# Vi-Sri/CerebralSignalNetworks

Hardware: AMD Instinct MI355X
Metric: EEG-segments/sec training (128ch x 500, hidden=768) (higher is better)
Workload: dtype bf16

## Files before the change

### cerebralsignalnetworks_amd/cabi.py

```python
import ctypes
import os

import torch

_HERE = os.path.dirname(os.path.abspath(__file__))
LIB_PATH = os.environ.get("CSN_LIB_PATH") or os.path.join(_HERE, "lib", "libcsn_hip.so")

CSN_F32, CSN_BF16 = 0, 1
STATUS_TIMEOUT, STATUS_NONFINITE, STATUS_STALE_SLOT = 1, 2, 4
ABI_VERSION = 6
LSTM_STATE = 0x100
LSTM_DROPOUT = 0x200
LSTM_REVERSE = 0x400
LSTM_RESIDENT = 0x800
RESIDENT_MAX_H = 128
TOPK_MERGE_STAGED_MAX = 2048
GRAD_OVERWRITE, GRAD_ACCUMULATE = 0, 1
SEG_DECAYED, SEG_SCALED = 1, 2

_c_void_p, _c_int, _c_i64, _c_size_t, _c_float = (ctypes.c_void_p, ctypes.c_int, ctypes.c_int64,
                                                  ctypes.c_size_t, ctypes.c_float)
_c_double = ctypes.c_double


# ... 410 lines not shown
        _check(load().csn_lstm_plan_set_io(self._plan, int(y_all_pitch), int(dy_all_pitch), int(bool(dx_add))))
        self._io = (int(y_all_pitch), int(dy_all_pitch), bool(dx_add))

    def _pitched(self, t, pitch, name):
        d = self.desc
        _need_cuda(t)
        pitch = pitch or d.H
        if (t.dtype != torch.float32 or tuple(t.shape) != (d.B, d.T, d.H) or t.stride() != (d.T * pitch, pitch, 1)
                or t.data_ptr() % 16):
            raise CsnError(f"LSTM {name}: a float32 [B,T,H] view with pitch {pitch} is needed, got {t.dtype} "
                           f"{tuple(t.shape)} strides {t.stride()}")
        return t

    def set_dropout(self, p, seed=0, subsequence=0):
        _check(load().csn_lstm_plan_set_dropout(self._plan, float(p), int(seed) & 0xFFFFFFFFFFFFFFFF,
                                                int(subsequence) & 0xFFFFFFFF))

    def dgates_copies(self):
        return load().csn_lstm_plan_dgates_copies(self._plan)

    def half_tile_launches(self, which):
        return load().csn_lstm_plan_half_tile_launches(self._plan, which)

    def forward(self, x_bti, w_ih, w_hh, b_ih, b_hh, want_all=False, h0=None, c0=None, want_state=False, y_all=None,
                state_out=None):
        d = self.desc
        _need_cuda(x_bti)
        if x_bti.dtype != torch.float32 or x_bti.stride(2) != 1:
            x_bti = x_bti.float().contiguous()
        want = (d.B, d.T, d.I) if self._views is None else self._views + (d.I,)
        assert x_bti.shape == want, (tuple(x_bti.shape), want)
        y_last = torch.empty((d.B, d.H), dtype=torch.float32, device=x_bti.device)
        if y_all is not None:
            y_all = self._pitched(y_all, self._io[0], "y_all")
        elif want_all:
            if self._io[0]:
                raise CsnError("LSTM y_all: the plan has a y_all pitch set (set_io): pass the view to write into")
            y_all = torch.empty((d.B, d.T, d.H), dtype=torch.float32, device=x_bti.device)
        ws = [[p.detach() for p in group] for group in (w_ih, w_hh, b_ih, b_hh)]
        for group in ws:
            for p in group:
                assert p.dtype == torch.float32 and p.is_contiguous() and p.is_cuda
        h0, c0 = self._state_in(h0), self._state_in(c0)
        if want_state and state_out is not None:
            h_n, c_n = state_out
            for out in state_out:
# ... 434 lines not shown
```

### cerebralsignalnetworks_amd/csrc/csn_common.h

```cpp
#pragma once
#include <hip/hip_runtime.h>
#include <stdint.h>
#include <stdio.h>
#include <stdlib.h>
#include <atomic>
#include <string>

#include "../../include/csn_hip.h"

namespace csn {

typedef __bf16 bf16_t;
typedef __attribute__((ext_vector_type(8))) __bf16 bf16x8;
typedef __attribute__((ext_vector_type(4))) __bf16 bf16x4;
typedef __attribute__((ext_vector_type(4))) float f32x4;
typedef __attribute__((ext_vector_type(4))) short s16x4;

void set_error(const std::string& msg);
int fail(int status, const char* fmt, ...);

#define CSN_HIP_CHECK(expr)                                                              \
  do {                                                                                   \
    hipError_t _e = (expr);                                                              \
    if (_e != hipSuccess)                                                                \
      return ::csn::fail(CSN_ERR_HIP, "%s failed: %s (%s:%d)", #expr, hipGetErrorString(_e), \
                         __FILE__, __LINE__);                                            \
  } while (0)

#define CSN_LAUNCH_CHECK()                                                               \
  do {                                                                                   \
    hipError_t _e = hipGetLastError();                                                   \
    if (_e != hipSuccess)                                                                \
      return ::csn::fail(CSN_ERR_HIP, "kernel launch failed: %s (%s:%d)",                \
                         hipGetErrorString(_e), __FILE__, __LINE__);                     \
  } while (0)

#define CSN_REQUIRE(cond, ...)                                                           \
  do {                                                                                   \
    if (!(cond)) return ::csn::fail(CSN_ERR_INVALID_ARGUMENT, __VA_ARGS__);              \
  } while (0)

struct Options {
  bool cell_v1, no_persist, no_persist_bwd, persist_streams, no_xcd_local, no_rotate, no_fuse_x, no_beside, beside_128,
      no_side_stream, fwd_ksplit, fwd_nsplit, fwd_flags, bwd_flags, dpoll_no_hint, fwd_hint, gemm_no_dma, gemm_no_256, gemm_generic, tn_no_tr, tn_no_stagger, filter_v1, tags_no_rearm, gemm_no_192, no_half_tiles, nt_no_w4, no_fwd_park;
  int chunk;
  int tn_stages;
};
static inline Options options_from_env() {
  auto on = [](const char* name) { return getenv(name) != nullptr; };
  auto num = [](const char* name, int dflt) {
    const char* e = getenv(name);
    return e ? atoi(e) : dflt;
  };
  Options o{};
  o.cell_v1 = on("CSN_CELL_V1");
  o.no_persist = on("CSN_NO_PERSIST");
  o.no_persist_bwd = on("CSN_NO_PERSIST_BWD");
  o.persist_streams = on("CSN_PERSIST_STREAMS");
  o.no_xcd_local = on("CSN_NO_XCD_LOCAL");
  o.no_rotate = on("CSN_NO_ROTATE");
  o.no_fuse_x = on("CSN_NO_FUSE_X");
  o.no_beside = on("CSN_NO_BESIDE");
  o.beside_128 = on("CSN_BESIDE_128");
  o.no_half_tiles = on("CSN_NO_HALF_TILES");
  o.no_fwd_park = on("CSN_NO_FWD_PARK");
  o.no_side_stream = on("CSN_NO_SIDE_STREAM");
  o.fwd_ksplit = on("CSN_FWD_KSPLIT");
  o.fwd_nsplit = on("CSN_FWD_NSPLIT");
  o.fwd_flags = on("CSN_FWD_FLAGS");
  o.bwd_flags = on("CSN_BWD_FLAGS");
  o.dpoll_no_hint = on("CSN_DPOLL_NO_HINT");
  o.fwd_hint = on("CSN_FWD_HINT");
  o.tn_no_stagger = on("CSN_TN_NO_STAGGER");
  o.gemm_no_dma = on("CSN_GEMM_NO_DMA");
  o.gemm_no_256 = on("CSN_GEMM_NO_256");
  o.gemm_no_192 = on("CSN_GEMM_NO_192");
  o.nt_no_w4 = on("CSN_NT_NO_W4");
  o.gemm_generic = on("CSN_GEMM_GENERIC");
  o.tn_no_tr = on("CSN_TN_NO_TR");
  o.filter_v1 = on("CSN_FILTER_V1");
#ifdef CSN_SLAB_TAGS
  o.tags_no_rearm = on("CSN_TAGS_NO_REARM");
#endif
  o.chunk = num("CSN_LSTM_CHUNK", 32);
  if (o.chunk < 1) o.chunk = 1;
  o.tn_stages = num("CSN_TN_STAGES", 4);
  return o;
}

static inline hipStream_t as_stream(csnStream_t s) { return reinterpret_cast<hipStream_t>(s); }
template <auto Kernel>
static int ensure_dyn_lds(int bytes) {
  static std::atomic<unsigned> done{0u};
// ... 68 lines not shown
```

### cerebralsignalnetworks_amd/csrc/lstm.hip

```cpp
#include <algorithm>
#include <cstring>
#include <vector>

#include "csn_common.h"
#include "lstm_cell_blk.h"
#include "lstm_cell_common.h"
#include "lstm_dropout.h"
#include "lstm_f32_persist.h"
#include "lstm_resident.h"

namespace csn {

struct LayerWs {
  size_t wih, whh, whht, wiht, whh_blk, whht_blk, bias, xproj, gates, c_all, h_all, dgates, dx, dc_carry, hblk[2],
      dgblk[2], h_blk_all, counters, dg_blk_all, bflags;
  size_t h_drop;
};
struct WsLayout {
  LayerWs layer[8];
  size_t x_c, x_blk, wih0_blk, dy_tm, tn_scratch, colsum, status, agree, agree_b, zeros_bh, f32_bias_part, total;
  size_t zero_fwd, zero_fwd_bytes, zero_bwd, zero_bwd_bytes;
  bool fuse_x;
  bool il, persist, persist_bwd;
  bool fwd_ns;
  bool f32_persist;
};

static bool whole_chip() {
  int dev = 0, cus = 0;
  if (hipGetDevice(&dev) != hipSuccess) return false;
  return hipDeviceGetAttribute(&cus, hipDeviceAttributeMultiprocessorCount, dev) == hipSuccess && cus >= 256;
}

static WsLayout make_layout(const csnLstmDesc& d, int training, bool dropout, const Options& opt) {
  WsLayout w{};
  w.il = cell_blk_supported(d.H, d.dtype, opt);
  const bool slabs_fit = ((size_t)d.T + 1) * (((size_t)d.B + 63) / 64 * 64) * (size_t)d.H * 8 < ((size_t)1 << 32);
  w.fwd_ns = w.il && fwd_ns_supported(d.B, d.H, d.dtype, opt) && d.L <= 4;
  w.persist = w.fwd_ns || (w.il && slabs_fit && fwd_persist_supported(d.B, d.H, d.dtype, opt) && d.L <= 4);
  w.persist_bwd = w.persist && slabs_fit && training && bwd_persist_supported(d.B, d.H, d.dtype, opt);
  size_t off = 0;
  const size_t es = dtype_size(d.dtype);
  auto take = [&](size_t bytes) {
// ... 56 lines not shown
    for (int l = 0; l < d.L; ++l) w.layer[l].h_blk_all = take(((size_t)d.T + 1) * Bpad * H * 4);
    if (training) {
      for (int l = 0; l < d.L; ++l) w.layer[l].dg_blk_all = take((size_t)d.T * Bpad * G * 4);
      w.zeros_bh = take((size_t)d.B * H * 4);
      w.f32_bias_part = take(MTt * 4 * G * 4);
      w.zero_bwd = off;
      for (int l = 0; l < d.L; ++l) w.layer[l].bflags = take((size_t)d.T * MTt * kF32FlagLine * 4);
      w.zero_bwd_bytes = off - w.zero_bwd;
    }
  }
  if (w.persist) {
    w.zero_fwd = off;
    for (int l = 0; l < d.L; ++l) w.layer[l].counters = take(((size_t)d.T + 1) * (Bpad / 64) * 4 * kPersistFlagLine * 4);
    w.agree = take(((size_t)d.T + 8) * 8 * sizeof(unsigned long long));
    w.zero_fwd_bytes = off - w.zero_fwd;
  }
  if (w.persist_bwd) {
    w.zero_bwd = off;
    for (int l = 0; l < d.L; ++l) {
      w.layer[l].dc_carry = take((size_t)d.B * H * 4);
      w.layer[l].bflags = take((size_t)d.T * (Bpad / 64) * 3 * kPersistFlagLine * 4);
    }
    w.agree_b = take(((size_t)d.T + 8) * 8 * sizeof(unsigned long long));
    w.zero_bwd_bytes = off - w.zero_bwd;
  }
  if (training) {
    w.dy_tm = take(TB * H * 4);
    w.tn_scratch = take(tn_bytes);
    w.colsum = take(colsum_scratch_bytes(G));
  }
  for (int l = 0; dropout && l + 1 < d.L; ++l) w.layer[l].h_drop = take(TB * H * es);
  w.total = off;
  return w;
}

static const int kPlanBits = CSN_LSTM_STATE | CSN_LSTM_DROPOUT | CSN_LSTM_REVERSE | CSN_LSTM_RESIDENT;

static int check_resident(const char* fn, const csnLstmDesc* d, int training) {
  if ((training & CSN_LSTM_RESIDENT) && !resident_supported(d->H))
    return fail(CSN_ERR_UNSUPPORTED, "%s: CSN_LSTM_RESIDENT takes H <= %d, not H=%d", fn, kResidentMaxH, d->H);
  return CSN_OK;
}
static void resident_options(Options& opt) {
  opt.cell_v1 = true;
  opt.no_persist = true;
}
// ... 259 lines not shown
  }
  CSN_HIP_CHECK(hipEventRecord(g_prof.pair[k][i], st));
  if (end) ++g_prof.pairs_used[k];
  return CSN_OK;
}

}

struct csnLstmPlan {
  csnLstmDesc d;
  int training;
  int dropout = 0;
  float drop_p = 0.f;
  uint64_t drop_seed = 0;
  uint32_t drop_subsequence = 0;
  int state;
  bool state_seen = false;
  int device;
  csn::Options opt;
  csn::WsLayout w;
  csn::SideCtx sc;
  csn::Prof prof;
  int dgates_copies = 0;
  int half_launches[2] = {0, 0};
  csnGradReadyFn grad_cb = nullptr;
  void* grad_cb_user = nullptr;
  int grad_accumulate = 0;
  int reverse = 0;
  int resident = 0;
  int64_t y_pitch = 0, dy_pitch = 0;
  int dx_add = 0;
  std::vector<int32_t> lengths;
  int t_eff = 0;
  int32_t* len_dev = nullptr;
  int32_t* len_pin = nullptr;
  hipEvent_t len_ev = nullptr;
  std::vector<int32_t> view_row, view_t0;
  int view_src_rows = 0, view_src_T = 0;
  int32_t* view_dev = nullptr;
  int32_t* view_pin = nullptr;
  hipEvent_t view_ev = nullptr;
  void grads_ready(int layer) const {
    if (grad_cb != nullptr) grad_cb(grad_cb_user, layer);
  }
};

// ... 41 lines not shown
    if (P->prof.ev[i]) (void)hipEventDestroy(P->prof.ev[i]);
  for (int k = 0; k < 2; ++k)
    for (hipEvent_t e : P->prof.pair[k]) (void)hipEventDestroy(e);
  if (P->len_ev) (void)hipEventDestroy(P->len_ev);
  if (P->len_pin) (void)hipHostFree(P->len_pin);
  if (P->len_dev) (void)hipFree(P->len_dev);
  if (P->view_ev) (void)hipEventDestroy(P->view_ev);
  if (P->view_pin) (void)hipHostFree(P->view_pin);
  if (P->view_dev) (void)hipFree(P->view_dev);
  if (switched) (void)hipSetDevice(cur);
  delete P;
}

extern "C" size_t csn_lstm_plan_workspace_bytes(const csnLstmPlan* P) { return P ? P->w.total : 0; }

extern "C" int csn_lstm_plan_path(const csnLstmPlan* P) {
  if (P == nullptr) return -1;
  if (P->resident) return 5;
  return P->w.f32_persist ? 4 : (P->w.persist_bwd ? 3 : (P->w.persist ? 2 : (P->w.il ? 1 : 0)));
}

extern "C" int csn_lstm_plan_dgates_copies(const csnLstmPlan* P) { return P == nullptr ? -1 : P->dgates_copies; }

extern "C" int csn_lstm_plan_half_tile_launches(const csnLstmPlan* P, int which) {
  return (P == nullptr || which < 0 || which > 1) ? -1 : P->half_launches[which];
}

static bool bwd_grouped(const csnLstmPlan* P, int T) {
  if (!P->w.persist_bwd) return false;
  const int MTg = (P->d.B + 63) / 64, nchg = (T + P->opt.chunk - 1) / P->opt.chunk;
  const int slots = P->d.L < nchg ? P->d.L : nchg;
  return slots <= 4 && slots * MTg <= 8 && !P->opt.persist_streams;
}

extern "C" const char* csn_lstm_plan_kernel_name(const csnLstmPlan* P, int which) {
  if (P == nullptr) return nullptr;
  const bool ks = (P->d.dtype == CSN_F32 ? P->d.H % 128 == 0 : P->d.H % 256 == 0);
  if (P->resident) return which == 0 ? "lstm_resident_fwd_kernel" : (which == 1 ? "lstm_resident_bwd_kernel" : nullptr);
  if (P->w.f32_persist) return which == 0 ? "lstm_fwd_f32_persist_kernel" : (which == 1 ? "lstm_bwd_f32_persist_kernel" : nullptr);
  if (which == 0) {
    if (P->w.fwd_ns) return "lstm_fwd_ns_kernel";
    if (P->w.persist) return "lstm_fwd_persist_kernel";
    if (P->w.il) return "lstm_cell_fwd_il_kernel";
    return ks ? "lstm_cell_fwd_ks_kernel" : "lstm_cell_fwd_kernel";
  }
  if (which == 1) {
// ... 1112 lines not shown
  const bool try_local = !P.opt.no_xcd_local;

  PersistBwdArgs a{};
  a.error_flag = (unsigned*)(ws + w.status);
  a.B = B; a.H = H; a.T = T; a.Bpad = Bpad; a.MT = MT;
  a.xcd_groups = 1;
  a.grid_slices = 32;
  a.beside_narrow = P.opt.beside_128 ? 1 : 0;
  a.rotate = !P.opt.no_rotate;
  a.data_polls = P.opt.bwd_flags ? 0 : (P.opt.dpoll_no_hint ? 2 : 1);
#ifdef CSN_SLAB_TAGS
  if (a.data_polls && P.opt.tags_no_rearm) a.data_polls |= 4;
#endif
  P.dgates_copies = 2;
  if (a.data_polls)
    for (int l = 0; l < NL; ++l) CSN_HIP_CHECK(hipMemsetAsync(ws + w.layer[l].dg_blk_all, 0xff, (size_t)4 * Bpad * G * 2, st));
  int n_launch = 0;
  P.half_launches[1] = 0;
  BesideGemm pending[3];
  DhAdd pending_add[3] = {{0, 0, 0}, {0, 0, 0}, {0, 0, 0}};
  DhAdd pending_drop[3] = {{0, 0, 0}, {0, 0, 0}, {0, 0, 0}};
  int npending = 0;
  if ((rc = prof_mark(g_prof, 2, st))) return rc;
  for (int dg = 0; dg < ndiag; ++dg) {
    int lay[4], chk[4], ns = 0;
    for (int l = NL - 1; l >= 0; --l) {
      const int c = dg - lag * (NL - 1 - l);
      if (c < 0 || c >= nch) continue;
      const LayerWs& L = w.layer[l];
      PersistBwdSlot& S = a.slot[ns];
      S.wt_blk = (const bf16_t*)(ws + L.whht_blk);
      S.gates = (const bf16_t*)(ws + L.gates);
      S.c_all = (const float*)(ws + L.c_all);
      if (l == NL - 1) {
        S.dy = A.dy_tm;
        S.dy_last = A.dy_tm ? nullptr : A.dy_last;
      } else {
        S.dy = (const float*)(ws + w.layer[l + 1].dx);
        S.dy_last = nullptr;
      }
      S.zeros = (const float*)(ws + w.zeros_bh);
      S.dc_carry = (float*)(ws + L.dc_carry);
      S.dgates = (bf16_t*)(ws + L.dgates);
      S.dg_blk_all = (bf16_t*)(ws + L.dg_blk_all);
      S.flags = (unsigned*)(ws + L.bflags);
      const Chunk k = chunk_at(C, c);
      S.t_hi = T - 1 - k.t0;
      S.nsteps = k.nsteps;
      lay[ns] = l;
      chk[ns] = c;
      ++ns;
    }
    if (ns == 0) {
      for (int i = 0; i < npending; ++i) {
        const BesideGemm& g = pending[i];
        if ((rc = gemm_nt(g.A, g.Bt, nullptr, g.C, g.M, g.N, g.K, CSN_BF16, CSN_F32, 0, st, P.opt))) return rc;
        if ((rc = drop_bwd(C, pending_drop[i].l - 1, pending_drop[i].t_lo, pending_drop[i].t_hi, st))) return rc;
        if (pending_add[i].l && (rc = add_dh_n(pending_add[i]))) return rc;
      }
      npending = 0;
      continue;
    }
    a.nslots = ns;
    a.ngemm = npending;
    const bool half = !P.opt.no_half_tiles && C.dlen == nullptr && 2 * ns * MT <= 8;
    a.half_tiles = half ? 1 : 0;
    a.MT = half ? 2 * MT : MT;
    if (half) {
      for (int i = 0; i < ns; ++i) a.slot[i].flags += (size_t)T * MT * kPersistFlagLine;
      ++P.half_launches[1];
    }
    DhAdd launch_adds[3], launch_drops[3];
    int nadds = 0;
    const int ndrops = npending;
    for (int i = 0; i < npending; ++i) {
      a.gemm[i] = pending[i];
      launch_drops[i] = pending_drop[i];
      if (pending_add[i].l) launch_adds[nadds++] = pending_add[i];
    }
    npending = 0;
    a.agree = try_local ? (unsigned long long*)(ws + w.agree_b) + (size_t)dg * 8 : nullptr;
    if ((rc = prof_pair(g_prof, 1, false, st))) return rc;
    if ((rc = launch_bwd_persist(a, st, C.dlen))) return rc;
    if ((rc = prof_pair(g_prof, 1, true, st))) return rc;
    ++n_launch;
    for (int i = 0; i < ndrops; ++i)
      if ((rc = drop_bwd(C, launch_drops[i].l - 1, launch_drops[i].t_lo, launch_drops[i].t_hi, st))) return rc;
    for (int i = 0; i < nadds; ++i)
      if ((rc = add_dh_n(launch_adds[i]))) return rc;
    for (int i = 0; i < ns; ++i) {
      const int l = lay[i];
      if (l == 0) continue;
      if (!beside) {
        if ((rc = dx_chunk_gemm(C, l, chk[i], dh_n, st))) return rc;
        continue;
      }
      const LayerWs& L = w.layer[l];
      const int t_hi = a.slot[i].t_hi, t_lo = t_hi - a.slot[i].nsteps + 1;
      pending_add[npending] = DhAdd{(dh_n && (chk[i] == 0 || C.dlen)) ? l : 0, t_lo, t_hi};
      pending_drop[npending] = DhAdd{l, t_lo, t_hi};
      pending[npending++] = BesideGemm{(const bf16_t*)(ws + L.dgates) + (size_t)t_lo * B * G, (const bf16_t*)(ws + L.wiht),
                                       (float*)(ws + L.dx) + (size_t)t_lo * B * H, (t_hi - t_lo + 1) * B, H, (int)G};
    }
  }
  if ((rc = prof_end(C, 1, n_launch, T * NL))) return rc;

  if (A.dx != nullptr && (rc = dx_out(C, A.dx, st))) return rc;
  for (int l = NL - 1; l >= 0; --l) {
    if ((rc = weight_grads_blk(C, A, l, st))) return rc;
    P.grads_ready(l);
  }
  return CSN_OK;
}

static int run_forward(Call& C, const FwdArgs& A) {
  if (C.P.resident) return forward_resident(C, A);
  if (C.w.persist) return forward_persist(C, A);
  if (C.w.il) return forward_il(C, A);
  if (C.w.f32_persist) return forward_f32p(C, A);
  return forward_v1(C, A);
}
static int run_backward(Call& C, const BwdArgs& A) {
  if (C.P.resident) return backward_resident(C, A);
  if (bwd_grouped(&C.P, C.T)) return backward_persist(C, A);
  if (C.w.il) return backward_il(C, A);
  if (C.w.f32_persist) return backward_f32p(C, A);
  return backward_v1(C, A);
}

static int check_state_args(const Plan& P, const char* fn, const void* const* ptrs, const char* const* names, int n) {
  for (int i = 0; i < n; ++i) {
    if (ptrs[i] == nullptr) continue;
    CSN_REQUIRE(P.state, "%s: %s given, but the plan was created without CSN_LSTM_STATE", fn, names[i]);
    CSN_REQUIRE((reinterpret_cast<uintptr_t>(ptrs[i]) & 15) == 0, "%s: %s must be 16-B aligned", fn, names[i]);
  }
  return CSN_OK;
}

static int gather_y_all_io(const Call& C, float* y_all) {
  const LayerWs& top = C.w.layer[C.NL - 1];
  const int64_t n = (int64_t)C.T_full * C.B * C.H, pitch = C.P.y_pitch ? C.P.y_pitch : C.H;
  if (C.dt == CSN_BF16)
    gather_y_all_io_kernel<bf16_t><<<grid_for(n), 256, 0, C.st>>>((const bf16_t*)(C.ws + top.h_all), y_all, C.dlen, C.B, C.T_full, C.H, pitch, C.P.reverse);
  else
    gather_y_all_io_kernel<float><<<grid_for(n), 256, 0, C.st>>>((const float*)(C.ws + top.h_all), y_all, C.dlen, C.B, C.T_full, C.H, pitch, C.P.reverse);
// ... 223 lines not shown
```

### cerebralsignalnetworks_amd/csrc/lstm_bwd_persist.hip

```cpp
#include "csn_common.h"
#include "lstm_cell_common.h"
#include "lstm_cell_blk.h"
#include "gemm_beside.h"

#ifdef CSN_PSTAMPS
#ifndef CSN_STAMP_BLOCK
#define CSN_STAMP_BLOCK 11
#endif
__device__ unsigned long long g_bstamps[16];
#define CSN_BSTAMP(i)                                                          \
  do {                                                                         \
    __builtin_amdgcn_sched_barrier(0);                                         \
    if (tid == 0 && blockIdx.x == CSN_STAMP_BLOCK) {                           \
      const unsigned long long now_ = wall_clock64();                          \
      atomicAdd(&g_bstamps[i], now_ - last_);                                  \
      last_ = now_;                                                            \
    }                                                                          \
    __builtin_amdgcn_sched_barrier(0);                                         \
  } while (0)
#else
#define CSN_BSTAMP(i)
#endif

namespace csn {
// ... 5 lines not shown
static constexpr int kBwdRedTile = 68;
__device__ __forceinline__ int bwd_red_pos(int r, int q) { return (r >> 1) + 8 * (r & 1) + 17 * q; }

typedef __attribute__((ext_vector_type(4))) unsigned bu32x4;

__device__ __forceinline__ bf16x8 bload_sc1_b128(__amdgpu_buffer_rsrc_t rsrc, unsigned byte_off, int soff = 0) {
  bu32x4 v = __builtin_amdgcn_raw_buffer_load_b128(rsrc, (int)byte_off, soff, 16);
  union { bu32x4 u; bf16x8 b; } cvt;
  cvt.u = v;
  return cvt.b;
}
template <bool WT>
__device__ __forceinline__ void bstore_b128(__amdgpu_buffer_rsrc_t rsrc, unsigned byte_off, const bf16x8& v, int soff = 0) {
  union { bu32x4 u; bf16x8 b; } cvt;
  cvt.b = v;
  __builtin_amdgcn_raw_buffer_store_b128(cvt.u, rsrc, (int)byte_off, soff, WT ? 16 : 0);
}

struct PersistLens { const int* lengths; };
struct PersistNoLens {};
template <bool MASK> struct PersistLensArg { typedef PersistNoLens type; };
template <> struct PersistLensArg<true> { typedef PersistLens type; };

template <int NUT, int KS, bool DPOLL, bool MASK = false, int RG = 4>
__global__ void __launch_bounds__(256) lstm_bwd_persist_kernel(PersistBwdArgs a, typename PersistLensArg<MASK>::type lens) {
#ifndef CSN_BWD_RING
#define CSN_BWD_RING 5
#endif
  constexpr int RING = KS >= 32 ? 3 : (KS < CSN_BWD_RING ? KS : CSN_BWD_RING);
  static_assert(RG == 4 || RG == 2, "tiles of 64 or 32 rows");
  constexpr int NT = RG * NUT;
  constexpr int QPR = 4 * NUT;
  constexpr int NPAIR = 16 * RG * QPR;
  constexpr int NPASS = NPAIR / 256;
  static_assert(NPAIR % 256 == 0, "tile must split evenly over the 256 threads");
  extern __shared__ __attribute__((aligned(16))) float4 red[];
  const int B = a.B, H = a.H, MT = a.MT, T = a.T;
  const int tid = threadIdx.x, lane = tid & 63, wave = tid >> 6;
#ifdef CSN_PSTAMPS
  const unsigned long long t_entry_ = wall_clock64();
#endif
  const int nslices = H / (16 * NUT);
  int grp, slice;
  if (a.xcd_groups) {
    grp = blockIdx.x & 7;
    slice = blockIdx.x >> 3;
    const int ngroups = a.nslots * MT, gs = a.grid_slices;
    if (grp >= ngroups || slice >= nslices) {
      if (a.ngemm > 0) {
        const int idle_here = gs - nslices;
        const unsigned base = grp <= ngroups ? (unsigned)(grp * idle_here)
                                             : (unsigned)(ngroups * idle_here + (grp - ngroups) * gs);
        const unsigned here = (unsigned)(grp < ngroups ? idle_here : gs);
        const unsigned local = (unsigned)(grp < ngroups ? slice - nslices : slice);
        const unsigned nworkers = (unsigned)(ngroups * idle_here + (8 - ngroups) * gs);
        for (int i = 0; i < a.ngemm; ++i)
          beside_gemm_tiles(a.gemm[i], reinterpret_cast<char*>(red), base, here, local, nworkers, ((a.gemm_wide >> i) & 1) != 0);
      }
      return;
    }
  } else {
    grp = blockIdx.x / nslices;
    slice = blockIdx.x % nslices;
  }
  const PersistBwdSlot& S = a.slot[grp / MT];
  const int mt = grp % MT;
  const int u0 = slice * 16 * NUT, m0 = mt * 16 * RG;
  const int K = 4 * H, kblocks = K >> 5;
  const int ks_beg = wave * KS;
  const size_t slab = (size_t)a.Bpad * K;
  const bf16_t* const wt_blk = S.wt_blk;
  const bf16_t* const gates = S.gates;
  const float* const c_all = S.c_all;
  const float* const dy = S.dy;
  const float* const dy_last = S.dy_last;
  bf16_t* const dgates = S.dgates;
  bf16_t* const dg_blk_all = S.dg_blk_all;
  unsigned* const flags = S.flags + (size_t)mt * kPersistFlagLine;
  const size_t flag_step = (size_t)MT * kPersistFlagLine;
  const int t_hi = S.t_hi, nsteps = S.nsteps;
  constexpr bool dpoll = DPOLL;

  bool local = false;
  if (a.xcd_groups && a.agree != nullptr) {
    if (tid == 0) {
      const unsigned xcc = __builtin_amdgcn_s_getreg(6164) & 7u;
      const unsigned long long mine = 1ull | (1ull << (8 + 6 * xcc));
      __hip_atomic_fetch_add(a.agree + grp, mine, __ATOMIC_RELAXED, __HIP_MEMORY_SCOPE_AGENT);
      const unsigned long long t_begin = wall_clock64();
      unsigned long long v;
      while (((v = __hip_atomic_load(a.agree + grp, __ATOMIC_RELAXED, __HIP_MEMORY_SCOPE_AGENT)) & 0xffull) <
             (unsigned long long)nslices) {
        __builtin_amdgcn_s_sleep(1);
        if (__hip_atomic_load(a.error_flag, __ATOMIC_RELAXED, __HIP_MEMORY_SCOPE_AGENT) != 0u) break;
        if (wall_clock64() - t_begin > kBwdSpinTimeoutTicks) {
          __hip_atomic_store(a.error_flag, 1u, __ATOMIC_RELAXED, __HIP_MEMORY_SCOPE_AGENT);
          break;
        }
      }
      ((__attribute__((address_space(3))) int*)(__attribute__((address_space(3))) void*)red)[0] = (int)(((v >> (8 + 6 * xcc)) & 63ull) == (unsigned long long)nslices);
    }
    __syncthreads();
    local = ((__attribute__((address_space(3))) int*)(__attribute__((address_space(3))) void*)red)[0] != 0;
// ... 16 lines not shown
  int plen[NPASS];
#pragma unroll
  for (int ps = 0; ps < NPASS; ++ps) {
    const int p = tid + ps * 256;
    prl[ps] = p / QPR;
    pjq[ps] = p % QPR;
    prow[ps] = m0 + prl[ps];
    puq[ps] = u0 + 4 * pjq[ps];
    pok[ps] = prow[ps] < B;
    dcn[ps] = make_float4(0.f, 0.f, 0.f, 0.f);
    cc[ps] = make_float4(0.f, 0.f, 0.f, 0.f);
    plen[ps] = 0;
    if constexpr (MASK) {
      if (pok[ps]) plen[ps] = lens.lengths[prow[ps]];
    }
    if (pok[ps]) {
      dcn[ps] = *reinterpret_cast<const float4*>(S.dc_carry + (size_t)prow[ps] * H + puq[ps]);
      cc[ps] = *reinterpret_cast<const float4*>(c_all + ((size_t)(t_hi + 1) * B + prow[ps]) * H + puq[ps]);
    }
  }

  bf16x8 gt_n[NPASS][2];
  float4 cpv_n[NPASS], dy_n[NPASS];
  auto request_saved = [&](int t) {
#pragma unroll
    for (int ps = 0; ps < NPASS; ++ps) {
      cpv_n[ps] = make_float4(0.f, 0.f, 0.f, 0.f);
      dy_n[ps] = make_float4(0.f, 0.f, 0.f, 0.f);
      if (pok[ps]) {
        const bf16x8* gp = reinterpret_cast<const bf16x8*>(gates + ((size_t)t * B + prow[ps]) * K + 4 * (size_t)puq[ps]);
        gt_n[ps][0] = nt_load(gp);
        gt_n[ps][1] = nt_load(gp + 1);
        cpv_n[ps] = nt_load(reinterpret_cast<const float4*>(c_all + ((size_t)t * B + prow[ps]) * H + puq[ps]));
        const float* dsrc = dy != nullptr ? dy + (size_t)t * B * H : ((dy_last != nullptr && t == T - 1) ? dy_last : S.zeros);
        dy_n[ps] = nt_load(reinterpret_cast<const float4*>(dsrc + (size_t)prow[ps] * H + puq[ps]));
      }
    }
  };
  request_saved(t_hi);
  const __amdgpu_buffer_rsrc_t ring_rsrc = __builtin_amdgcn_make_buffer_rsrc(
      (void*)dg_blk_all, 0, (int)((size_t)4 * slab * 2), 0x00020000);
  const int slab_bytes = (int)(slab * 2);
#ifdef CSN_PSTAMPS
  unsigned long long last_ = wall_clock64();
  if (tid == 0 && blockIdx.x == CSN_STAMP_BLOCK) atomicAdd(&g_bstamps[6], last_ - t_entry_);
#endif

  auto arm_region = [&](int arm_off) {
    const bf16x8 sent = __builtin_bit_cast(bf16x8, (u32x4){0xffffffffu, 0xffffffffu, 0xffffffffu, 0xffffffffu});
#pragma unroll
    for (int ps = 0; ps < NPASS; ++ps) {
      const unsigned o0 = (unsigned)(blk_offset(prow[ps], 4 * (int64_t)puq[ps], K) * 2);
      const unsigned o1 = (unsigned)(blk_offset(prow[ps], 4 * (int64_t)puq[ps] + 8, K) * 2);
      if (local) {
        bstore_b128<false>(ring_rsrc, o0, sent, arm_off);
        bstore_b128<false>(ring_rsrc, o1, sent, arm_off);
      } else {
        bstore_b128<true>(ring_rsrc, o0, sent, arm_off);
        bstore_b128<true>(ring_rsrc, o1, sent, arm_off);
      }
    }
  };
  for (int s = 0; s < nsteps; ++s) {
    const int t = t_hi - s;
    bf16x8 gt[NPASS][2];
    float4 cpv[NPASS], dyv[NPASS];
#pragma unroll
    for (int ps = 0; ps < NPASS; ++ps) {
      gt[ps][0] = gt_n[ps][0];
      gt[ps][1] = gt_n[ps][1];
      cpv[ps] = cpv_n[ps];
      dyv[ps] = dy_n[ps];
    }

    f32x4 acc[RG][NUT];
#pragma unroll
    for (int rg = 0; rg < RG; ++rg)
#pragma unroll
      for (int ut = 0; ut < NUT; ++ut) acc[rg][ut] = (f32x4){0.f, 0.f, 0.f, 0.f};

    if (t < T - 1) {
      {
        const int npw = nslices >> 2;
        const unsigned* fl;
        if constexpr (dpoll) {
// ... 113 lines not shown
                bool sentinel = false;
                int kbo2 = rot_t * 1024;
#pragma unroll 1
                for (int kb = 0; kb < KS; ++kb) {
#pragma unroll
                  for (int rg = 0; rg < RG; ++rg) {
                    const u32x4 u = __builtin_bit_cast(u32x4, bload_sc1_b128(slabs_rsrc, base + (unsigned)(rg * kblocks) * 1024u, src_off + kbo2));
                    sentinel |= (u[0] == 0xffffffffu) | (u[3] == 0xffffffffu);
                  }
                  kbo2 = kbo2 + 1024 == KS * 1024 ? 0 : kbo2 + 1024;
                }
                proven = !__any(sentinel);
              }
              again = __hip_atomic_load(a.error_flag, __ATOMIC_RELAXED, __HIP_MEMORY_SCOPE_AGENT) == 0u;
              if (wall_clock64() - t_phase > kBwdSpinTimeoutTicks) {
                __hip_atomic_store(a.error_flag, 1u, __ATOMIC_RELAXED, __HIP_MEMORY_SCOPE_AGENT);
                again = false;
              }
            }
          }
        }
      } while (again);
    }
    if (s + 1 < nsteps) request_saved(t - 1);
    __builtin_amdgcn_sched_barrier(0);
    CSN_BSTAMP(1);

#pragma unroll
    for (int rg = 0; rg < RG; ++rg)
#pragma unroll
      for (int ut = 0; ut < NUT; ++ut)
        red[(wave * NT + rg * NUT + ut) * kBwdRedTile + bwd_red_pos(lane & 15, lane >> 4)] = make_float4(acc[rg][ut][0], acc[rg][ut][1], acc[rg][ut][2], acc[rg][ut][3]);
    __syncthreads();
    CSN_BSTAMP(2);

    if (dpoll && !CSN_DPOLL_NO_REARM(a.data_polls)) {
      arm_region(__builtin_amdgcn_readfirstlane(((t + 2) & 3) * slab_bytes));
      __builtin_amdgcn_sched_barrier(0);
    }

    const __amdgpu_buffer_rsrc_t slabs_rsrc = dpoll ? ring_rsrc : __builtin_amdgcn_make_buffer_rsrc(
        (void*)(dg_blk_all + (size_t)t * slab), 0, slab_bytes, 0x00020000);
    const int dst_off = dpoll ? __builtin_amdgcn_readfirstlane((t & 3) * slab_bytes) : 0;
#pragma unroll
    for (int ps = 0; ps < NPASS; ++ps) {
      if (!pok[ps]) {
        if (dpoll) {
// ... 68 lines not shown
        bstore_b128<false>(slabs_rsrc, o0, lo, dst_off);
        bstore_b128<false>(slabs_rsrc, o1, hi, dst_off);
      } else {
        bstore_b128<true>(slabs_rsrc, o0, lo, dst_off);
        bstore_b128<true>(slabs_rsrc, o1, hi, dst_off);
      }
      bf16x8* op = reinterpret_cast<bf16x8*>(dgates + ((size_t)t * B + row) * K + 4 * (size_t)uq);
      nt_store(op, lo);
      nt_store(op + 1, hi);
      dcn[ps] = make_float4(dcarry[0], dcarry[1], dcarry[2], dcarry[3]);
      cc[ps] = cpv[ps];
    }
    CSN_BSTAMP(3);
    if (!dpoll) asm volatile("s_waitcnt vmcnt(0)" ::: "memory");
    __syncthreads();
    CSN_BSTAMP(4);
    if (!dpoll && tid == 0) {
      unsigned* fl = flags + (size_t)t * flag_step + slice;
      if (local) *fl = 1u;
      else __hip_atomic_store(fl, 1u, __ATOMIC_RELAXED, __HIP_MEMORY_SCOPE_AGENT);
    }
    CSN_BSTAMP(5);
  }

#pragma unroll
  for (int ps = 0; ps < NPASS; ++ps)
    if (pok[ps]) *reinterpret_cast<float4*>(S.dc_carry + (size_t)prow[ps] * H + puq[ps]) = dcn[ps];
}

bool bwd_persist_supported(int B, int H, int dtype, const Options& opt) {
  if (dtype != CSN_BF16 || opt.no_persist || opt.no_persist_bwd) return false;
  return H == 128 || H == 256 || H == 384 || H == 512 || H == 768 || H == 1024;
}
int bwd_persist_slices(int H) { return H / 32; }

template <int NUT, int KS>
static int launch_bwd_persist_t(const PersistBwdArgs& a, hipStream_t st, const int* lengths) {
  size_t lds = (size_t)4 * (a.half_tiles ? 2 : 4) * NUT * kBwdRedTile * sizeof(float4);
  if (lengths != nullptr) {
    if (int rc = ensure_dyn_lds<&lstm_bwd_persist_kernel<NUT, KS, false, true>>((int)kBesideLdsBytes)) return rc;
    if (int rc = ensure_dyn_lds<&lstm_bwd_persist_kernel<NUT, KS, true, true>>((int)kBesideLdsBytes)) return rc;
  } else if (a.half_tiles) {
    if (int rc = ensure_dyn_lds<&lstm_bwd_persist_kernel<NUT, KS, false, false, 2>>((int)kBesideLdsBytes)) return rc;
    if (int rc = ensure_dyn_lds<&lstm_bwd_persist_kernel<NUT, KS, true, false, 2>>((int)kBesideLdsBytes)) return rc;
  } else {
    if (int rc = ensure_dyn_lds<&lstm_bwd_persist_kernel<NUT, KS, false>>((int)kBesideLdsBytes)) return rc;
// ... 16 lines not shown
  const unsigned grid = b.xcd_groups ? 8u * (unsigned)b.grid_slices : nslices * (unsigned)(b.MT * b.nslots);
  if (lengths != nullptr) {
    const PersistLens pl{lengths};
    if (b.data_polls) lstm_bwd_persist_kernel<NUT, KS, true, true><<<dim3(grid), 256, lds, st>>>(b, pl);
    else lstm_bwd_persist_kernel<NUT, KS, false, true><<<dim3(grid), 256, lds, st>>>(b, pl);
  } else if (b.half_tiles) {
    if (b.data_polls) lstm_bwd_persist_kernel<NUT, KS, true, false, 2><<<dim3(grid), 256, lds, st>>>(b, PersistNoLens{});
    else lstm_bwd_persist_kernel<NUT, KS, false, false, 2><<<dim3(grid), 256, lds, st>>>(b, PersistNoLens{});
  } else if (b.data_polls) lstm_bwd_persist_kernel<NUT, KS, true><<<dim3(grid), 256, lds, st>>>(b, PersistNoLens{});
  else lstm_bwd_persist_kernel<NUT, KS, false><<<dim3(grid), 256, lds, st>>>(b, PersistNoLens{});
  CSN_LAUNCH_CHECK();
  return CSN_OK;
}

int launch_bwd_persist(const PersistBwdArgs& a, hipStream_t st, const int* lengths) {
  CSN_REQUIRE(a.nslots >= 1 && a.nslots <= 4 && a.MT >= 1, "launch_bwd_persist: bad slot count");
  const int ns = bwd_persist_slices(a.H);
  CSN_REQUIRE(ns % 4 == 0 && ns <= kPersistFlagLine, "launch_bwd_persist: H=%d gives %d slices", a.H, ns);
  if (a.xcd_groups) CSN_REQUIRE(a.nslots * a.MT <= 8, "launch_bwd_persist: groups do not fit 8 XCDs");
  CSN_REQUIRE(a.MT * (a.half_tiles ? 32 : 64) == a.Bpad, "launch_bwd_persist: %d tiles of %d rows are not Bpad=%d", a.MT,
              a.half_tiles ? 32 : 64, a.Bpad);
  CSN_REQUIRE(!a.half_tiles || (a.xcd_groups && lengths == nullptr), "launch_bwd_persist: 32-row groups need the grouped form and no lengths");
  CSN_REQUIRE(a.ngemm >= 0 && a.ngemm <= 3 && (a.ngemm == 0 || a.xcd_groups), "launch_bwd_persist: bad GEMM list");
  for (int i = 0; i < a.ngemm; ++i)
    CSN_REQUIRE(a.gemm[i].K % 64 == 0 && a.gemm[i].K <= (1 << 22) && a.gemm[i].N % 4 == 0 && a.gemm[i].M > 0, "launch_bwd_persist: GEMM %d shape", i);
  switch (a.H) {
    case 1024: return launch_bwd_persist_t<2, 32>(a, st, lengths);
    case 768: return launch_bwd_persist_t<2, 24>(a, st, lengths);
    case 512: return launch_bwd_persist_t<2, 16>(a, st, lengths);
    case 384: return launch_bwd_persist_t<2, 12>(a, st, lengths);
    case 256: return launch_bwd_persist_t<2, 8>(a, st, lengths);
    case 128: return launch_bwd_persist_t<2, 4>(a, st, lengths);
  }
  return fail(CSN_ERR_UNSUPPORTED, "launch_bwd_persist: no kernel for H=%d", a.H);
}

}

#ifdef CSN_PSTAMPS
extern "C" int csn_debug_read_bstamps(unsigned long long* out) {
  unsigned long long z[16] = {0};
  if (hipMemcpyFromSymbol(out, HIP_SYMBOL(g_bstamps), sizeof(z)) != hipSuccess) return 1;
  if (hipMemcpyToSymbol(HIP_SYMBOL(g_bstamps), z, sizeof(z)) != hipSuccess) return 1;
  return 0;
}
#endif
// ... 1 lines not shown
```

### cerebralsignalnetworks_amd/csrc/lstm_cell_blk.h

```cpp
#pragma once
#include "csn_common.h"

#ifdef CSN_SLAB_TAGS
#define CSN_DPOLL_MODE(x) ((x) & 3)
#define CSN_DPOLL_NO_REARM(x) (((x) & 4) != 0)
#else
#define CSN_DPOLL_MODE(x) (x)
#define CSN_DPOLL_NO_REARM(x) false
#endif

namespace csn {

struct CellFwdProb {
  const bf16_t* h_prev_blk;
  const bf16_t* w_blk;
  const float* xproj;
  const float* c_prev;
  bf16_t* gates_out;
  float* c_out;
  bf16_t* h_out;
  bf16_t* h_out_blk;
};
struct CellFwdArgs {
  CellFwdProb p[4];
// ... 55 lines not shown
static constexpr int kParkSlots = 6;
constexpr size_t fwd_persist_lds_bytes(int nq, bool park) {
  return (size_t)(4 * 4 * nq * kRedTile + 4 * nq + (park ? kParkSlots * 256 : 0)) * 16;
}
bool fwd_persist_supported(int B, int H, int dtype, const Options& opt);
bool fwd_ns_supported(int B, int H, int dtype, const Options& opt);
int fwd_ns_slices(int H);
int launch_fwd_ns(const PersistFwdArgs& a, hipStream_t st);
int fwd_persist_slices(int H);
int launch_fwd_persist(const PersistFwdArgs& a, hipStream_t st);

struct PersistBwdSlot {
  const bf16_t* wt_blk;
  const bf16_t* gates;
  const float* c_all;
  const float* dy;
  const float* dy_last;
  const float* zeros;
  float* dc_carry;
  bf16_t* dgates;
  bf16_t* dg_blk_all;
  unsigned* flags;
  int t_hi, nsteps;
};
struct PersistBwdArgs {
  PersistBwdSlot slot[4];
  int nslots;
  BesideGemm gemm[3];
  int ngemm;
  int beside_narrow;
  int gemm_wide;
  int grid_slices;
  int xcd_groups;
  int rotate;
  int data_polls;
  unsigned long long* agree;
  unsigned* error_flag;
  int B, H, T, Bpad, MT;
  int half_tiles;
};
bool bwd_persist_supported(int B, int H, int dtype, const Options& opt);
int bwd_persist_slices(int H);
int launch_bwd_persist(const PersistBwdArgs& a, hipStream_t st, const int* lengths = nullptr);

enum { kPrepBlockify = 0, kPrepPermRows, kPrepTransPerm, kPrepBias, kPrepCastX, kPrepBlockifyX };
static constexpr int kPrepMaxJobs = 32;
struct PrepJob {
  int kind;
  const float* a;
  const float* b;
  void* dst;
  int64_t n0, n1, n2, s0, s1, H;
  int perm_r, perm_k;
  int64_t work;
  unsigned blk_begin, blk_count;
  const int* len;
};
struct PrepArgs {
  PrepJob job[kPrepMaxJobs];
  int njobs;
  const int* vrow;
  const int* vt0;
};
// ... 17 lines not shown
```

Baseline: 27740.

## Merge steady-state backward diagonal launches into one multi-round persistent kernel

In the backward wavefront, the diagonals where every layer is active are folded into a single persistent launch that runs several rounds. Global atomic counters replace the kernel boundaries: recurrent blocks publish per-round completion, and side-GEMM worker blocks wait on them, then publish their own completion for the next layer. The aim is to remove per-chunk launch overhead and the tail drain between launches. In exchange it adds spin-wait dependencies, extra kernel-argument reads, and more constraints on when the path is taken (no dropout, no lengths, full chunks only).

Result: faster. 28070 (median of 6 runs) (+1.2%).

```diff
diff --git a/cerebralsignalnetworks_amd/cabi.py b/cerebralsignalnetworks_amd/cabi.py
--- a/cerebralsignalnetworks_amd/cabi.py
+++ b/cerebralsignalnetworks_amd/cabi.py
@@ -456,6 +456,11 @@
     def half_tile_launches(self, which):
         return load().csn_lstm_plan_half_tile_launches(self._plan, which)
 
+    def bwd_launches(self, which):
+        fn = load().csn_lstm_plan_bwd_launches
+        fn.restype, fn.argtypes = _c_int, [_c_void_p, _c_int]
+        return int(fn(self._plan, which))
+
     def forward(self, x_bti, w_ih, w_hh, b_ih, b_hh, want_all=False, h0=None, c0=None, want_state=False, y_all=None,
                 state_out=None):
         d = self.desc
diff --git a/cerebralsignalnetworks_amd/csrc/csn_common.h b/cerebralsignalnetworks_amd/csrc/csn_common.h
--- a/cerebralsignalnetworks_amd/csrc/csn_common.h
+++ b/cerebralsignalnetworks_amd/csrc/csn_common.h
@@ -42,7 +42,7 @@
 
 struct Options {
   bool cell_v1, no_persist, no_persist_bwd, persist_streams, no_xcd_local, no_rotate, no_fuse_x, no_beside, beside_128,
-      no_side_stream, fwd_ksplit, fwd_nsplit, fwd_flags, bwd_flags, dpoll_no_hint, fwd_hint, gemm_no_dma, gemm_no_256, gemm_generic, tn_no_tr, tn_no_stagger, filter_v1, tags_no_rearm, gemm_no_192, no_half_tiles, nt_no_w4, no_fwd_park;
+      no_side_stream, fwd_ksplit, fwd_nsplit, fwd_flags, bwd_flags, dpoll_no_hint, fwd_hint, gemm_no_dma, gemm_no_256, gemm_generic, tn_no_tr, tn_no_stagger, filter_v1, tags_no_rearm, gemm_no_192, no_half_tiles, nt_no_w4, no_fwd_park, bwd_no_merge;
   int chunk;
   int tn_stages;
 };
@@ -69,6 +69,7 @@
   o.fwd_nsplit = on("CSN_FWD_NSPLIT");
   o.fwd_flags = on("CSN_FWD_FLAGS");
   o.bwd_flags = on("CSN_BWD_FLAGS");
+  o.bwd_no_merge = on("CSN_BWD_NO_MERGE");
   o.dpoll_no_hint = on("CSN_DPOLL_NO_HINT");
   o.fwd_hint = on("CSN_FWD_HINT");
   o.tn_no_stagger = on("CSN_TN_NO_STAGGER");
diff --git a/cerebralsignalnetworks_amd/csrc/lstm.hip b/cerebralsignalnetworks_amd/csrc/lstm.hip
--- a/cerebralsignalnetworks_amd/csrc/lstm.hip
+++ b/cerebralsignalnetworks_amd/csrc/lstm.hip
@@ -18,7 +18,7 @@
 };
 struct WsLayout {
   LayerWs layer[8];
-  size_t x_c, x_blk, wih0_blk, dy_tm, tn_scratch, colsum, status, agree, agree_b, zeros_bh, f32_bias_part, total;
+  size_t x_c, x_blk, wih0_blk, dy_tm, tn_scratch, colsum, status, agree, agree_b, merge_cnt, zeros_bh, f32_bias_part, total;
   size_t zero_fwd, zero_fwd_bytes, zero_bwd, zero_bwd_bytes;
   bool fuse_x;
   bool il, persist, persist_bwd;
@@ -121,6 +121,7 @@
       w.layer[l].bflags = take((size_t)d.T * (Bpad / 64) * 3 * kPersistFlagLine * 4);
     }
     w.agree_b = take(((size_t)d.T + 8) * 8 * sizeof(unsigned long long));
+    w.merge_cnt = take((2 * (size_t)d.L * d.T * sizeof(unsigned) + 15) / 16 * 16);
     w.zero_bwd_bytes = off - w.zero_bwd;
   }
   if (training) {
@@ -426,6 +427,7 @@
   csn::SideCtx sc;
   csn::Prof prof;
   int dgates_copies = 0;
+  int bwd_launches[2] = {0, 0};
   int half_launches[2] = {0, 0};
   csnGradReadyFn grad_cb = nullptr;
   void* grad_cb_user = nullptr;
@@ -513,6 +515,9 @@
 
 extern "C" int csn_lstm_plan_dgates_copies(const csnLstmPlan* P) { return P == nullptr ? -1 : P->dgates_copies; }
 
+extern "C" int csn_lstm_plan_bwd_launches(const csnLstmPlan* P, int which) {
+  return (P == nullptr || which < 0 || which > 1) ? -1 : P->bwd_launches[which];
+}
 extern "C" int csn_lstm_plan_half_tile_launches(const csnLstmPlan* P, int which) {
   return (P == nullptr || which < 0 || which > 1) ? -1 : P->half_launches[which];
 }
@@ -1671,8 +1676,14 @@
   DhAdd pending_drop[3] = {{0, 0, 0}, {0, 0, 0}, {0, 0, 0}};
   int npending = 0;
   if ((rc = prof_mark(g_prof, 2, st))) return rc;
+  const int m_first = lag * (NL - 1), m_count = nch - m_first;
+  const bool merge = beside && !P.opt.bwd_no_merge && a.data_polls && C.dlen == nullptr && !drop_on(C) && dh_n == nullptr && m_count >= 2;
+  unsigned* const cnt = (unsigned*)(ws + w.merge_cnt);
+  P.bwd_launches[0] = P.bwd_launches[1] = 0;
   for (int dg = 0; dg < ndiag; ++dg) {
     int lay[4], chk[4], ns = 0;
+    const bool merged = merge && dg == m_first;
+    if (merged) dg = m_first + m_count - 1;
     for (int l = NL - 1; l >= 0; --l) {
       const int c = dg - lag * (NL - 1 - l);
       if (c < 0 || c >= nch) continue;
@@ -1696,9 +1707,33 @@
       const Chunk k = chunk_at(C, c);
       S.t_hi = T - 1 - k.t0;
       S.nsteps = k.nsteps;
+      S.cnt_pub = S.cnt_wait = -1;
       lay[ns] = l;
       chk[ns] = c;
       ++ns;
+    }
+    a.nrounds = 1;
+    a.chunk = Cz;
+    a.cnt = cnt;
+    if (merged) {
+      CSN_REQUIRE(ns == NL && npending == NL - 1, "backward_persist: merged launch without every layer");
+      a.nrounds = m_count;
+      for (int i = 0; i < ns; ++i) {
+        PersistBwdSlot& S = a.slot[i];
+        const int c0 = chk[i] - (m_count - 1);
+        S.t_hi += (m_count - 1) * Cz;
+        S.nsteps = Cz;
+        if (lay[i] > 0) S.cnt_pub = lay[i] * nch + c0;
+        if (lay[i] < NL - 1) S.cnt_wait = (NL + lay[i] + 1) * nch + c0;
+      }
+      for (int i = 0; i < npending; ++i) CSN_REQUIRE(pending[i].M == Cz * B, "backward_persist: merged launch with a short GEMM");
+      a.wk_wait = a.slot[0].cnt_pub - 1;
+      a.wk_pub = a.slot[1].cnt_wait + 1;
+      a.wk_stride = nch + lag;
+      for (int i = 1; i + 1 < ns; ++i)
+        CSN_REQUIRE(a.slot[i].cnt_pub == a.slot[0].cnt_pub - i * a.wk_stride && a.slot[i + 1].cnt_wait == a.slot[1].cnt_wait - i * a.wk_stride,
+                    "backward_persist: merged launch whose counters are not evenly spaced");
+      P.bwd_launches[1] = m_count;
     }
     if (ns == 0) {
       for (int i = 0; i < npending; ++i) {
@@ -1717,7 +1752,7 @@
     a.MT = half ? 2 * MT : MT;
     if (half) {
       for (int i = 0; i < ns; ++i) a.slot[i].flags += (size_t)T * MT * kPersistFlagLine;
-      ++P.half_launches[1];
+      P.half_launches[1] += merged ? m_count : 1;
     }
     DhAdd launch_adds[3], launch_drops[3];
     int nadds = 0;
@@ -1733,6 +1768,12 @@
     if ((rc = launch_bwd_persist(a, st, C.dlen))) return rc;
     if ((rc = prof_pair(g_prof, 1, true, st))) return rc;
     ++n_launch;
+    if (merged)
+      for (int i = 0; i < ns; ++i) {
+        const Chunk k = chunk_at(C, chk[i]);
+        a.slot[i].t_hi = T - 1 - k.t0;
+        a.slot[i].nsteps = k.nsteps;
+      }
     for (int i = 0; i < ndrops; ++i)
       if ((rc = drop_bwd(C, launch_drops[i].l - 1, launch_drops[i].t_lo, launch_drops[i].t_hi, st))) return rc;
     for (int i = 0; i < nadds; ++i)
@@ -1752,6 +1793,7 @@
                                        (float*)(ws + L.dx) + (size_t)t_lo * B * H, (t_hi - t_lo + 1) * B, H, (int)G};
     }
   }
+  P.bwd_launches[0] = n_launch;
   if ((rc = prof_end(C, 1, n_launch, T * NL))) return rc;
 
   if (A.dx != nullptr && (rc = dx_out(C, A.dx, st))) return rc;
@@ -1770,6 +1812,7 @@
   return forward_v1(C, A);
 }
 static int run_backward(Call& C, const BwdArgs& A) {
+  C.P.bwd_launches[0] = C.P.bwd_launches[1] = 0;
   if (C.P.resident) return backward_resident(C, A);
   if (bwd_grouped(&C.P, C.T)) return backward_persist(C, A);
   if (C.w.il) return backward_il(C, A);
diff --git a/cerebralsignalnetworks_amd/csrc/lstm_bwd_persist.hip b/cerebralsignalnetworks_amd/csrc/lstm_bwd_persist.hip
--- a/cerebralsignalnetworks_amd/csrc/lstm_bwd_persist.hip
+++ b/cerebralsignalnetworks_amd/csrc/lstm_bwd_persist.hip
@@ -51,6 +51,37 @@
 template <bool MASK> struct PersistLensArg { typedef PersistNoLens type; };
 template <> struct PersistLensArg<true> { typedef PersistLens type; };
 
+__device__ __forceinline__ bool round_leader() {
+  unsigned t = threadIdx.x;
+  asm volatile("" : "+v"(t));
+  return t == 0u;
+}
+__device__ __forceinline__ void round_publish(unsigned* word) {
+  asm volatile("s_waitcnt vmcnt(0)" ::: "memory");
+  __syncthreads();
+  if (round_leader()) {
+    __builtin_amdgcn_fence(__ATOMIC_RELEASE, "agent");
+    asm volatile("s_waitcnt vmcnt(0)" ::: "memory");
+    __hip_atomic_fetch_add(word, 1u, __ATOMIC_RELAXED, __HIP_MEMORY_SCOPE_AGENT);
+  }
+}
+__device__ __forceinline__ void round_wait(const unsigned* word, unsigned want, unsigned* error_flag) {
+  if (round_leader()) {
+    const unsigned long long t_begin = wall_clock64();
+    while (__hip_atomic_load(word, __ATOMIC_RELAXED, __HIP_MEMORY_SCOPE_AGENT) < want) {
+      __builtin_amdgcn_s_sleep(1);
+      if (__hip_atomic_load(error_flag, __ATOMIC_RELAXED, __HIP_MEMORY_SCOPE_AGENT) != 0u) break;
+      if (wall_clock64() - t_begin > kBwdSpinTimeoutTicks) {
+        __hip_atomic_store(error_flag, 1u, __ATOMIC_RELAXED, __HIP_MEMORY_SCOPE_AGENT);
+        break;
+      }
+    }
+    __builtin_amdgcn_fence(__ATOMIC_ACQUIRE, "agent");
+    asm volatile("s_waitcnt vmcnt(0)" ::: "memory");
+  }
+  __syncthreads();
+}
+
 template <int NUT, int KS, bool DPOLL, bool MASK = false, int RG = 4>
 __global__ void __launch_bounds__(256) lstm_bwd_persist_kernel(PersistBwdArgs a, typename PersistLensArg<MASK>::type lens) {
 #ifndef CSN_BWD_RING
@@ -70,27 +101,52 @@
   const unsigned long long t_entry_ = wall_clock64();
 #endif
   const int nslices = H / (16 * NUT);
+  unsigned bid = blockIdx.x;
+  if (a.xcd_groups) {
+    const int wgrp = (int)(bid & 7u), wslice = (int)(bid >> 3);
+    const int ngroups = a.nslots * MT, gs = a.grid_slices;
+    if (wgrp >= ngroups || wslice >= nslices) {
+      if (a.ngemm > 0) {
+        const int idle_here = gs - nslices;
+        const unsigned base = wgrp <= ngroups ? (unsigned)(wgrp * idle_here)
+                                              : (unsigned)(ngroups * idle_here + (wgrp - ngroups) * gs);
+        const unsigned here = (unsigned)(wgrp < ngroups ? idle_here : gs);
+        const unsigned local = (unsigned)(wgrp < ngroups ? wslice - nslices : wslice);
+        const unsigned nworkers = (unsigned)(ngroups * idle_here + (8 - ngroups) * gs);
+        typedef const PersistBwdArgs __attribute__((address_space(4)))* KArgs;
+        KArgs ap = (KArgs)__builtin_amdgcn_kernarg_segment_ptr();
+        for (int r = 0;; ++r) {
+          asm volatile("" : "+s"(ap));
+          if (r >= ap->nrounds) break;
+          for (int i = 0;; ++i) {
+            asm volatile("" : "+s"(ap));
+            if (i >= ap->ngemm) break;
+            BesideGemm g;
+            g.A = ap->gemm[i].A; g.Bt = ap->gemm[i].Bt; g.C = ap->gemm[i].C;
+            g.M = ap->gemm[i].M; g.N = ap->gemm[i].N; g.K = ap->gemm[i].K;
+            if (r > 0) {
+              round_wait(ap->cnt + (ap->wk_wait + r - i * ap->wk_stride), (unsigned)(ap->MT * nslices), ap->error_flag);
+              const unsigned down = (unsigned)(r * ap->chunk) * (unsigned)ap->B;
+              g.A -= (size_t)down * (unsigned)g.K;
+              g.C -= (size_t)down * (unsigned)g.N;
+            }
+            beside_gemm_tiles(g, reinterpret_cast<char*>(red), base, here, local, nworkers, ((ap->gemm_wide >> i) & 1) != 0);
+            asm volatile("" : "+s"(ap));
+            if (r + 1 < ap->nrounds) round_publish(ap->cnt + (ap->wk_pub + r - i * ap->wk_stride));
+          }
+        }
+      }
+      return;
+    }
+  }
+  asm volatile("" : "+s"(bid));
   int grp, slice;
   if (a.xcd_groups) {
-    grp = blockIdx.x & 7;
-    slice = blockIdx.x >> 3;
-    const int ngroups = a.nslots * MT, gs = a.grid_slices;
-    if (grp >= ngroups || slice >= nslices) {
-      if (a.ngemm > 0) {
-        const int idle_here = gs - nslices;
-        const unsigned base = grp <= ngroups ? (unsigned)(grp * idle_here)
-                                             : (unsigned)(ngroups * idle_here + (grp - ngroups) * gs);
-        const unsigned here = (unsigned)(grp < ngroups ? idle_here : gs);
-        const unsigned local = (unsigned)(grp < ngroups ? slice - nslices : slice);
-        const unsigned nworkers = (unsigned)(ngroups * idle_here + (8 - ngroups) * gs);
-        for (int i = 0; i < a.ngemm; ++i)
-          beside_gemm_tiles(a.gemm[i], reinterpret_cast<char*>(red), base, here, local, nworkers, ((a.gemm_wide >> i) & 1) != 0);
-      }
-      return;
-    }
+    grp = (int)(bid & 7u);
+    slice = (int)(bid >> 3);
   } else {
-    grp = blockIdx.x / nslices;
-    slice = blockIdx.x % nslices;
+    grp = (int)bid / nslices;
+    slice = (int)bid % nslices;
   }
   const PersistBwdSlot& S = a.slot[grp / MT];
   const int mt = grp % MT;
@@ -107,7 +163,7 @@
   bf16_t* const dg_blk_all = S.dg_blk_all;
   unsigned* const flags = S.flags + (size_t)mt * kPersistFlagLine;
   const size_t flag_step = (size_t)MT * kPersistFlagLine;
-  const int t_hi = S.t_hi, nsteps = S.nsteps;
+  int t_hi = S.t_hi, nsteps = S.nsteps;
   constexpr bool dpoll = DPOLL;
 
   bool local = false;
@@ -170,7 +226,7 @@
 
   bf16x8 gt_n[NPASS][2];
   float4 cpv_n[NPASS], dy_n[NPASS];
-  auto request_saved = [&](int t) {
+  auto request_saved = [&](int t, const float* dy) {
 #pragma unroll
     for (int ps = 0; ps < NPASS; ++ps) {
       cpv_n[ps] = make_float4(0.f, 0.f, 0.f, 0.f);
@@ -185,7 +241,6 @@
       }
     }
   };
-  request_saved(t_hi);
   const __amdgpu_buffer_rsrc_t ring_rsrc = __builtin_amdgcn_make_buffer_rsrc(
       (void*)dg_blk_all, 0, (int)((size_t)4 * slab * 2), 0x00020000);
   const int slab_bytes = (int)(slab * 2);
@@ -209,6 +264,22 @@
       }
     }
   };
+  typedef const PersistBwdArgs __attribute__((address_space(4)))* KArgs;
+  KArgs ap = (KArgs)__builtin_amdgcn_kernarg_segment_ptr();
+  for (int r = 0;; ++r) {
+  if (KS < 32 && r > 0) {
+    asm volatile("" : "+s"(ap));
+    const int cnt_wait = ap->slot[grp / ap->MT].cnt_wait;
+    if (cnt_wait >= 0) {
+      const int gs = ap->grid_slices, ngroups = ap->nslots * ap->MT;
+      round_wait(ap->cnt + (cnt_wait + r), (unsigned)(ngroups * (gs - nslices) + (8 - ngroups) * gs), ap->error_flag);
+    }
+  }
+  {
+    const float* dy_r = dy;
+    asm volatile("" : "+s"(dy_r));
+    request_saved(t_hi, dy_r);
+  }
   for (int s = 0; s < nsteps; ++s) {
     const int t = t_hi - s;
     bf16x8 gt[NPASS][2];
@@ -368,7 +439,7 @@
         }
       } while (again);
     }
-    if (s + 1 < nsteps) request_saved(t - 1);
+    if (s + 1 < nsteps) request_saved(t - 1, dy);
     __builtin_amdgcn_sched_barrier(0);
     CSN_BSTAMP(1);
 
@@ -483,6 +554,14 @@
     }
     CSN_BSTAMP(5);
   }
+  if (KS >= 32) break;
+  asm volatile("" : "+s"(ap));
+  if (r + 1 >= ap->nrounds) break;
+  const int cnt_pub = ap->slot[grp / ap->MT].cnt_pub;
+  if (cnt_pub >= 0) round_publish(ap->cnt + (cnt_pub + r));
+  t_hi -= nsteps;
+  nsteps = t_hi + 1 < ap->chunk ? t_hi + 1 : ap->chunk;
+  }
 
 #pragma unroll
   for (int ps = 0; ps < NPASS; ++ps)
@@ -545,6 +624,9 @@
               a.half_tiles ? 32 : 64, a.Bpad);
   CSN_REQUIRE(!a.half_tiles || (a.xcd_groups && lengths == nullptr), "launch_bwd_persist: 32-row groups need the grouped form and no lengths");
   CSN_REQUIRE(a.ngemm >= 0 && a.ngemm <= 3 && (a.ngemm == 0 || a.xcd_groups), "launch_bwd_persist: bad GEMM list");
+  CSN_REQUIRE(a.nrounds == 1 || (a.nrounds > 1 && a.xcd_groups && a.data_polls && lengths == nullptr && a.ngemm == a.nslots - 1 &&
+                                 a.ngemm >= 1 && a.H < 1024 && a.chunk >= 1 && a.cnt != nullptr),
+              "launch_bwd_persist: a merged launch needs the grouped form with data polls, no lengths and a GEMM per layer boundary");
   for (int i = 0; i < a.ngemm; ++i)
     CSN_REQUIRE(a.gemm[i].K % 64 == 0 && a.gemm[i].K <= (1 << 22) && a.gemm[i].N % 4 == 0 && a.gemm[i].M > 0, "launch_bwd_persist: GEMM %d shape", i);
   switch (a.H) {
diff --git a/cerebralsignalnetworks_amd/csrc/lstm_cell_blk.h b/cerebralsignalnetworks_amd/csrc/lstm_cell_blk.h
--- a/cerebralsignalnetworks_amd/csrc/lstm_cell_blk.h
+++ b/cerebralsignalnetworks_amd/csrc/lstm_cell_blk.h
@@ -101,6 +101,7 @@
   bf16_t* dg_blk_all;
   unsigned* flags;
   int t_hi, nsteps;
+  int cnt_pub, cnt_wait;
 };
 struct PersistBwdArgs {
   PersistBwdSlot slot[4];
@@ -117,7 +118,11 @@
   unsigned* error_flag;
   int B, H, T, Bpad, MT;
   int half_tiles;
+  int nrounds, chunk;
+  unsigned* cnt;
+  int wk_wait, wk_pub, wk_stride;
 };
+static_assert(sizeof(PersistBwdArgs) <= 4096, "PersistBwdArgs is passed by value: the kernel-argument segment holds 4096 bytes");
 bool bwd_persist_supported(int B, int H, int dtype, const Options& opt);
 int bwd_persist_slices(int H);
 int launch_bwd_persist(const PersistBwdArgs& a, hipStream_t st, const int* lengths = nullptr);
```
